# edexheim/como

Measured on AMD Instinct MI355X. Metric: GN iters/sec, 8-keyframe 640x480 photometric BA, higher is better.
Workload: dtype f64

## Files before the change

como_amd/csrc/densify.hip:

```cpp
#include "select.cuh"
#include "../../include/como_hip.h"

namespace como {

template <typename T> int select_hist(const T*, const uint8_t*, long, int, uint32_t*, int, hipStream_t);

template <typename T> struct Q4 { T x, y, z, w; };
template <typename T>
__device__ __forceinline__ Q4<T> ld4(const T* __restrict__ p) {
  Q4<T> v;
  if constexpr (sizeof(T) == 4) {
    const float4 f = *reinterpret_cast<const float4*>(p);
    v.x = f.x; v.y = f.y; v.z = f.z; v.w = f.w;
  } else {
    const double2 a = *reinterpret_cast<const double2*>(p);
    const double2 b = *reinterpret_cast<const double2*>(p + 2);
    v.x = a.x; v.y = a.y; v.z = b.x; v.w = b.y;
  }
  return v;
}

template <typename T>
__global__ __launch_bounds__(256) void dense_ref_kernel(
    const T* __restrict__ Kt, long kt_slot_stride, const int* __restrict__ pixidx, const T* __restrict__ logzm,
    const T* __restrict__ Twc, const T* __restrict__ Kmat, const T* __restrict__ dlogzm_dTwc, int n, int m, int Wimg,
    T* __restrict__ Pwn, T* __restrict__ dPwn_dTwc, T* __restrict__ uvec, T* __restrict__ zbuf, T* __restrict__ logzn_out,
    uint32_t* __restrict__ hists, const int* __restrict__ pixcoord, int compact) {
  using KeyT = typename KeyOf<T>::type;
  __shared__ uint32_t lh[SEL_BINS];
  __shared__ T coef[64][8];
  const int b = blockIdx.y;
  for (int k = threadIdx.x; k < SEL_BINS; k += 256) lh[k] = 0;
  for (int k = threadIdx.x; k < 64 * 8; k += 256) {
    const int j = k >> 3, e = k & 7;
    T v = T(0);
    if (j < m) {
      if (e == 0) v = logzm[(long)b * m + j];
      else if (e < 7) v = dlogzm_dTwc[((long)b * m + j) * 6 + (e - 1)];
    }
    coef[j][e] = v;
  }
  T Tm[12];
#pragma unroll
  for (int k = 0; k < 12; ++k) Tm[k] = Twc[16 * (long)b + k];
  const T fx = Kmat[0], fy = Kmat[4], cx = Kmat[2], cy = Kmat[5];
  __syncthreads();
  const int stride = gridDim.x * 256;
  const int iters = (n + stride - 1) / stride;
  for (int it = 0; it < iters; ++it) {
    const int i0 = it * stride + blockIdx.x * 256 + threadIdx.x;
    const bool inr = i0 < n;
    const int i = inr ? i0 : n - 1;
// ... 13 lines not shown
    const T z = exp(logz);
    const int crow = pixcoord ? pixcoord[(long)b * n + i] : row;
    T rx, ry;
    {
#pragma clang fp contract(off)
      rx = (T(crow % Wimg) - cx) / fx;
      ry = (T(crow / Wimg) - cy) / fy;
    }
    const T Xc = z * rx, Yc = z * ry, Zc = z;
    T Xw, Yw, Zw;
    rigid_apply(Tm, Xc, Yc, Zc, Xw, Yw, Zw);
    const T u0 = Tm[0] * Xc + Tm[1] * Yc + Tm[2] * Zc;
    const T u1 = Tm[4] * Xc + Tm[5] * Yc + Tm[6] * Zc;
    const T u2 = Tm[8] * Xc + Tm[9] * Yc + Tm[10] * Zc;
    if (inr && Pwn && compact) {
      const long base3 = (long)b * 3 * n + i, base6 = (long)b * 6 * n + i;
      Pwn[base3] = Xw; Pwn[base3 + n] = Yw; Pwn[base3 + 2 * (long)n] = Zw;
#pragma unroll
      for (int k = 0; k < 6; ++k) dPwn_dTwc[base6 + (long)k * n] = acc[1 + k];
    } else if (inr && Pwn) {
      const long base3 = (long)b * 3 * n + i, base18 = (long)b * 18 * n + i;
      Pwn[base3] = Xw; Pwn[base3 + n] = Yw; Pwn[base3 + 2 * (long)n] = Zw;
      uvec[base3] = u0; uvec[base3 + n] = u1; uvec[base3 + 2 * (long)n] = u2;
      const T uu[3] = {u0, u1, u2};
#pragma unroll
      for (int r = 0; r < 3; ++r) {
        const T r0 = Tm[r * 4 + 0], r1 = Tm[r * 4 + 1], r2 = Tm[r * 4 + 2];
        const T s0 = -(r1 * Zc - r2 * Yc), s1 = -(r2 * Xc - r0 * Zc), s2 = -(r0 * Yc - r1 * Xc);
        dPwn_dTwc[base18 + (long)(r * 6 + 0) * n] = s0 + uu[r] * acc[1];
        dPwn_dTwc[base18 + (long)(r * 6 + 1) * n] = s1 + uu[r] * acc[2];
        dPwn_dTwc[base18 + (long)(r * 6 + 2) * n] = s2 + uu[r] * acc[3];
        dPwn_dTwc[base18 + (long)(r * 6 + 3) * n] = r0 + uu[r] * acc[4];
        dPwn_dTwc[base18 + (long)(r * 6 + 4) * n] = r1 + uu[r] * acc[5];
        dPwn_dTwc[base18 + (long)(r * 6 + 5) * n] = r2 + uu[r] * acc[6];
      }
    }
    if (inr) {
      zbuf[(long)b * n + i] = Zc;
      if (logzn_out) logzn_out[(long)b * n + i] = logz;
    }
    sel_lds_add(lh, sel_digit<KeyT>(abs_key(Zc), 0), inr);
  }
  __syncthreads();
  if (hists) sel_flush(lh, hists + (long)b * 6 * SEL_BINS);
}

template <typename T> struct DAcc { typedef T type __attribute__((ext_vector_type(4))); };
__device__ __forceinline__ typename DAcc<float>::type d_mfma(float a, float b, typename DAcc<float>::type c) {
  return __builtin_amdgcn_mfma_f32_16x16x4f32(a, b, c, 0, 0, 0);
}
__device__ __forceinline__ typename DAcc<double>::type d_mfma(double a, double b, typename DAcc<double>::type c) {
  return __builtin_amdgcn_mfma_f64_16x16x4f64(a, b, c, 0, 0, 0);
}
template <typename T> __device__ __forceinline__ int d_mfma_row(int lane, int reg);
template <> __device__ __forceinline__ int d_mfma_row<float>(int lane, int reg) { return (lane >> 4) * 4 + reg; }
template <> __device__ __forceinline__ int d_mfma_row<double>(int lane, int reg) { return (lane >> 4) + 4 * reg; }

__device__ __forceinline__ void wave_lds_fence() {
  __builtin_amdgcn_fence(__ATOMIC_RELEASE, "workgroup");
  __builtin_amdgcn_wave_barrier();
  __builtin_amdgcn_fence(__ATOMIC_ACQUIRE, "workgroup");
}

template <typename T>
struct DRFuse {
  const int* ref_pairs;
  int np_max;
  const T* pair_T;
  const T* pair_aff;
  const T* vals;
  const T* img_base;
  const long* tgt_img;
  T* r_out;
  uint8_t* valid_out;
  uint32_t* rhists;
  int H, W, anorm_f32;
};

template <typename T, bool FUSE>
__global__ __launch_bounds__(256) void dense_ref_mfma_kernel(
    const T* __restrict__ Kt, long kt_slot_stride, const int* __restrict__ pixidx, const T* __restrict__ logzm,
    const T* __restrict__ Twc, const T* __restrict__ Kmat, const T* __restrict__ dlogzm_dTwc, int n, int m,
    int Wimg, T* __restrict__ Pwn, T* __restrict__ dPwn_dTwc, T* __restrict__ uvec, T* __restrict__ zbuf,
    T* __restrict__ logzn_out, uint32_t* __restrict__ hists, const int* __restrict__ pixcoord, int compact, DRFuse<T> fz) {
  using KeyT = typename KeyOf<T>::type;
  using acc_t = typename DAcc<T>::type;
  __shared__ uint32_t lh[SEL_BINS];
  __shared__ uint32_t lh2[FUSE ? SEL_BINS : 1];
  __shared__ T sD[4][64 * 9];
  if constexpr (FUSE) {
    for (int k = threadIdx.x; k < SEL_BINS; k += 256) lh2[k] = 0;
  }
  const int b = blockIdx.y, tid = threadIdx.x, lane = tid & 63, wv = tid >> 6, c = lane & 15, q = lane >> 4;
  for (int k = tid; k < SEL_BINS; k += 256) lh[k] = 0;
  T bop[16];
#pragma unroll
  for (int se = 0; se < 16; ++se) {
    const int k = 16 * (se >> 2) + 4 * q + (se & 3);
    T v = T(0);
    if (k < m) {
      if (c == 0) v = logzm[(long)b * m + k];
      else if (c < 7) v = dlogzm_dTwc[((long)b * m + k) * 6 + (c - 1)];
    }
    bop[se] = v;
  }
  T Tm[12];
#pragma unroll
  for (int k = 0; k < 12; ++k) Tm[k] = Twc[16 * (long)b + k];
  const T fx = Kmat[0], fy = Kmat[4], cx = Kmat[2], cy = Kmat[5];
  __syncthreads();
  T* myD = sD[wv];
  const int tiles = (n + 63) >> 6;
  Q4<T> kA[2][4], kB[2][4];
  auto load_half = [&](Q4<T> (&dst)[2][4], int tile_, int half) {
#pragma unroll
    for (int h2 = 0; h2 < 2; ++h2) {
      const int ii = min((tile_ << 6) + 16 * (2 * half + h2) + c, n - 1);
      const int rw = pixidx ? pixidx[(long)b * n + ii] : ii;
      const T* Kr = Kt + (long)b * kt_slot_stride + (long)rw * m;
#pragma unroll
      for (int s = 0; s < 4; ++s) {
        const int kk = min(16 * s + 4 * q, m - 4);
        dst[h2][s] = ld4(Kr + kk);
      }
    }
  };
  auto mma_half = [&](const Q4<T> (&src)[2][4], int half) {
#pragma unroll
    for (int h2 = 0; h2 < 2; ++h2) {
      acc_t acc = {T(0), T(0), T(0), T(0)};
#pragma unroll
      for (int s = 0; s < 4; ++s) {
        acc = d_mfma(src[h2][s].x, bop[4 * s + 0], acc);
        acc = d_mfma(src[h2][s].y, bop[4 * s + 1], acc);
        acc = d_mfma(src[h2][s].z, bop[4 * s + 2], acc);
        acc = d_mfma(src[h2][s].w, bop[4 * s + 3], acc);
      }
      if (c < 8) {
#pragma unroll
        for (int r = 0; r < 4; ++r) myD[(16 * (2 * half + h2) + d_mfma_row<T>(lane, r)) * 9 + c] = acc[r];
      }
    }
  };
  const int tstride = gridDim.x * 4;
  int tile = blockIdx.x * 4 + wv;
  if (tile < tiles) load_half(kA, tile, 0);
  for (; tile < tiles; tile += tstride) {
    const int px0 = tile << 6;
    load_half(kB, tile, 1);
    mma_half(kA, 0);
    if (tile + tstride < tiles) load_half(kA, tile + tstride, 0);
    mma_half(kB, 1);
    wave_lds_fence();
    T a7[7];
#pragma unroll
    for (int a = 0; a < 7; ++a) a7[a] = myD[lane * 9 + a];
    wave_lds_fence();
    const int i0 = px0 + lane;
    const bool inr = i0 < n;
    const int i = inr ? i0 : n - 1;
    const int row = pixidx ? pixidx[(long)b * n + i] : i;
    const T logz = a7[0];
    const T z = exp(logz);
    const int crow = pixcoord ? pixcoord[(long)b * n + i] : row;
    T rx, ry;
    {
#pragma clang fp contract(off)
      rx = (T(crow % Wimg) - cx) / fx;
      ry = (T(crow / Wimg) - cy) / fy;
    }
    const T Xc = z * rx, Yc = z * ry, Zc = z;
    T Xw, Yw, Zw;
    rigid_apply(Tm, Xc, Yc, Zc, Xw, Yw, Zw);
    const T u0 = Tm[0] * Xc + Tm[1] * Yc + Tm[2] * Zc;
    const T u1 = Tm[4] * Xc + Tm[5] * Yc + Tm[6] * Zc;
    const T u2 = Tm[8] * Xc + Tm[9] * Yc + Tm[10] * Zc;
    if (inr && Pwn && compact) {
      const long base3 = (long)b * 3 * n + i, base6 = (long)b * 6 * n + i;
      Pwn[base3] = Xw; Pwn[base3 + n] = Yw; Pwn[base3 + 2 * (long)n] = Zw;
#pragma unroll
      for (int k = 0; k < 6; ++k) dPwn_dTwc[base6 + (long)k * n] = a7[1 + k];
    } else if (inr && Pwn) {
      const long base3 = (long)b * 3 * n + i, base18 = (long)b * 18 * n + i;
      Pwn[base3] = Xw; Pwn[base3 + n] = Yw; Pwn[base3 + 2 * (long)n] = Zw;
      uvec[base3] = u0; uvec[base3 + n] = u1; uvec[base3 + 2 * (long)n] = u2;
      const T uu[3] = {u0, u1, u2};
#pragma unroll
      for (int r = 0; r < 3; ++r) {
        const T r0 = Tm[r * 4 + 0], r1 = Tm[r * 4 + 1], r2 = Tm[r * 4 + 2];
        const T s0 = -(r1 * Zc - r2 * Yc), s1 = -(r2 * Xc - r0 * Zc), s2 = -(r0 * Yc - r1 * Xc);
        dPwn_dTwc[base18 + (long)(r * 6 + 0) * n] = s0 + uu[r] * a7[1];
        dPwn_dTwc[base18 + (long)(r * 6 + 1) * n] = s1 + uu[r] * a7[2];
        dPwn_dTwc[base18 + (long)(r * 6 + 2) * n] = s2 + uu[r] * a7[3];
        dPwn_dTwc[base18 + (long)(r * 6 + 3) * n] = r0 + uu[r] * a7[4];
        dPwn_dTwc[base18 + (long)(r * 6 + 4) * n] = r1 + uu[r] * a7[5];
        dPwn_dTwc[base18 + (long)(r * 6 + 5) * n] = r2 + uu[r] * a7[6];
      }
    }
    if (inr) {
      zbuf[(long)b * n + i] = Zc;
      if (logzn_out) logzn_out[(long)b * n + i] = logz;
    }
    sel_lds_add(lh, sel_digit<KeyT>(abs_key(Zc), 0), inr);
    if constexpr (FUSE) {
      const T vr = fz.vals[(long)b * n + i];
      const T ax = fz.anorm_f32 ? (T)(1.0f / (float)fz.W) : T(1) / T(fz.W), ay = fz.anorm_f32 ? (T)(1.0f / (float)fz.H) : T(1) / T(fz.H);
      for (int q = 0; q < fz.np_max; ++q) {
        const int p = fz.ref_pairs[(long)b * fz.np_max + q];
        if (p < 0) break;
        const T* M = fz.pair_T + 12 * (long)p;
        const T scale = fz.pair_aff[2 * p], bias = fz.pair_aff[2 * p + 1];
        const T* img = fz.img_base + fz.tgt_img[p];
        T X, Y, Z;
        rigid_apply(M, Xw, Yw, Zw, X, Y, Z);
        const T pu = project1(fx, X, Z, cx);
        const T pv = project1(fy, Y, Z, cy);
        const bool ok = in_image(pu, pv, fz.H, fz.W) && (Z > T(0));
        Taps<T> t = make_taps(grid_position(pu, fz.W, ax), grid_position(pv, fz.H, ay), fz.H, fz.W);
        const T It = tap_sum(img, t);
        const T r = It - scale * vr + bias;
        if (inr) {
          const long oi = (long)p * n + i;
          fz.r_out[oi] = r;
          fz.valid_out[oi] = ok ? 1 : 0;
        }
        sel_lds_add(lh2, sel_digit<KeyT>(abs_key(r), 0), inr && ok);
      }
    }
  }
  __syncthreads();
  if (hists) sel_flush(lh, hists + (long)b * 6 * SEL_BINS);
  if constexpr (FUSE) sel_flush(lh2, fz.rhists);
}

template <typename T>
__global__ void copy_elems_kernel(const T* __restrict__ src, T* __restrict__ dst, int n) {
  const int i = blockIdx.x * blockDim.x + threadIdx.x;
  if (i < n) dst[i] = src[i];
}

template <typename T>
__global__ __launch_bounds__(256) void depth_band_kernel(
    const T* __restrict__ Kt, long kt_slot_stride, const T* __restrict__ logzm, const T* __restrict__ logzm_prev, int rows, int m,
    T* __restrict__ lref, T* __restrict__ err, T* __restrict__ l1, float* __restrict__ l1max, const T* __restrict__ med_prev3,
    T* __restrict__ zbuf, uint32_t* __restrict__ hists, unsigned* __restrict__ ncand, int init) {
  using KeyT = typename KeyOf<T>::type;
  __shared__ uint32_t lh[SEL_BINS];
  __shared__ T coef[64];
  __shared__ T sdelta, sabs;
  const int b = blockIdx.y;
  for (int k = threadIdx.x; k < SEL_BINS; k += 256) lh[k] = 0;
  if (threadIdx.x < 64) {
    const int k = threadIdx.x;
    const T cur = (k < m) ? logzm[(long)b * m + k] : T(0);
    const T prv = (k < m && !init) ? logzm_prev[(long)b * m + k] : cur;
    coef[k] = cur;
    T d = fabs(cur - prv), a = fabs(cur);
#pragma unroll
    for (int off = 32; off > 0; off >>= 1) { d = fmax(d, __shfl_xor(d, off, 64)); a = fmax(a, __shfl_xor(a, off, 64)); }
    if (k == 0) { sdelta = d; sabs = a; }
  }
  __syncthreads();
  const T eps = (sizeof(T) == 4) ? T(4e-6) : T(4e-15);
  const T delta = sdelta * (T(1) + T(64) * eps) + (sdelta > T(0) ? eps : T(0));
  const T mp = init ? T(0) : log(med_prev3[3 * b]);
  const T band = init ? T(0) : (T)l1max[b] * delta + eps * (fabs(mp) + T(1));
  const T inf = (T)__builtin_inff();
  const int stride = gridDim.x * 256;
  unsigned mycand = 0;
  float myl1max = 0.f;
  for (int i0 = blockIdx.x * 256 + threadIdx.x; i0 - (int)threadIdx.x < rows; i0 += stride) {
    const bool inr = i0 < rows;
    const int i = inr ? i0 : rows - 1;
    const long si = (long)b * rows + i;
    bool cand = init != 0;
    T e = T(0), lr = T(0), rl1 = T(0);
    if (!init) {
      rl1 = l1[si];
      lr = lref[si];
      e = err[si] + rl1 * delta;
      cand = !((lr + e < mp - band) || (lr - e > mp + band));
    }
    T z;
    if (cand) {
      const T* Kr = Kt + (long)b * kt_slot_stride + (long)i * m;
      T acc = T(0), s1 = T(0);
// ... 185 lines not shown
  using acc_t = typename KAcc<T>::type;
  __shared__ T sK[64 * 65];
  __shared__ T sx[64 * 2];
  __shared__ T sE[64 * 4];
  const int b = blockIdx.y;
  for (int k = threadIdx.x; k < 64 * 64; k += 256) {
    const int r = k >> 6, c = k & 63;
    sK[r * 65 + c] = (r < m && c < m) ? Kinv[(long)b * m * m + (long)r * m + c] : T(0);
  }
  for (int k = threadIdx.x; k < 64 * 2; k += 256) sx[k] = (k < m * 2) ? xm[(long)b * m * 2 + k] : T(0);
  for (int k = threadIdx.x; k < 64 * 4; k += 256) sE[k] = (k < m * 4) ? Em[(long)b * m * 4 + k] : ((k & 3) == 0 || (k & 3) == 3 ? T(1) : T(0));
  __syncthreads();
  const long np = (long)Hp * Wp;
  const T ar = T(1) / T(Hc), ac = T(1) / T(Wc);
  const int lane = threadIdx.x & 63, wv = threadIdx.x >> 6, px = lane & 15, kq = lane >> 4;
  const long groups = (np + 15) / 16;
  for (long grp = (long)blockIdx.x * 4 + wv; grp < groups; grp += (long)gridDim.x * 4) {
    const long p = min(grp * 16 + px, np - 1);
    const int row = (int)(p / Wp), col = (int)(p % Wp);
    T rn, cn;
    {
#pragma clang fp contract(off)
      rn = (T(2) * ar) * T(row) + ar - T(1);
      cn = (T(2) * ac) * T(col) + ac - T(1);
    }
    T En[4];
    cov_lookup(cov + (long)b * 4 * Hc * Wc, Hc, Wc, rn, cn, En);
    T a[16];
#pragma unroll
    for (int s2 = 0; s2 < 16; ++s2) {
      const int k = 4 * s2 + kq;
      const T v = kernel_py(rn, cn, En, sx[2 * k], sx[2 * k + 1], sE + 4 * k) * scale;
      a[s2] = (k < m) ? v : T(0);
    }
#pragma unroll
    for (int t = 0; t < 4; ++t) {
      if (16 * t >= m) break;
      acc_t acc = {T(0), T(0), T(0), T(0)};
#pragma unroll
      for (int s2 = 0; s2 < 16; ++s2) acc = k_mfma(a[s2], sK[(4 * s2 + kq) * 65 + 16 * t + px], acc);
      const int j = 16 * t + px;
#pragma unroll
      for (int r = 0; r < 4; ++r) {
        const long pr = grp * 16 + k_mfma_row<T>(lane, r);
        if (pr < np && j < m) {
          out[((long)b * np + pr) * m + j] = acc[r];
          if (out32) out32[((long)b * np + pr) * m + j] = (float)acc[r];
        }
      }
    }
  }
}

template <typename T>
int dense_ref(const T* Kt, long kt_slot_stride, const int* pixidx, const T* logzm, const T* Twc, const T* Kmat,
              const T* dlogzm_dTwc, int B, int n, int m, int Wimg, T* Pwn, T* dPwn_dTwc, T* uvec, T* zbuf, T* logzn_out,
              void* hists_v, T* med_out3, const int* pixcoord, int flags, hipStream_t s, const DRFuse<T>* fuse = nullptr) {
  using KeyT = typename KeyOf<T>::type;
  const int compact = (flags & 16) ? 1 : 0;
  const bool depth_only = (flags & 8) != 0;
  if (!Kt || !logzm || !Twc || !Kmat || !dlogzm_dTwc || !zbuf || !hists_v || !med_out3 ||
      B <= 0 || n <= 0 || m <= 0 || m > 64 || (m & 3) || Wimg <= 0)
    return COMO_ERR_ARG;
  if (depth_only) { Pwn = nullptr; dPwn_dTwc = nullptr; uvec = nullptr; }
  else if (!Pwn || !dPwn_dTwc || (!uvec && !compact)) return COMO_ERR_ARG;
  uint32_t* hists = (uint32_t*)hists_v;
  if (!(flags & 4)) {
  if ((flags & 64) && (flags & 2)) hists = nullptr;
  if (hists && !(flags & 1) && !zero_words(hists, (size_t)B * 6 * SEL_BINS, s))
    return COMO_ERR_LAUNCH;
  int gx = (n + 255) / 256;
  if (gx > 512) gx = 512;
  if (sizeof(T) == 4 || (!depth_only && !(flags & 32))) {
    int gm = ((n + 63) / 64 + 3) / 4;
    if (gm > 256) gm = 256;
    if (fuse && !depth_only)
      hipLaunchKernelGGL((dense_ref_mfma_kernel<T, true>), dim3(gm, B), dim3(256), 0, s, Kt, kt_slot_stride, pixidx, logzm, Twc, Kmat,
                         dlogzm_dTwc, n, m, Wimg, Pwn, dPwn_dTwc, uvec, zbuf, logzn_out, hists, pixcoord, compact, *fuse);
    else
      hipLaunchKernelGGL((dense_ref_mfma_kernel<T, false>), dim3(gm, B), dim3(256), 0, s, Kt, kt_slot_stride, pixidx, logzm, Twc, Kmat,
                         dlogzm_dTwc, n, m, Wimg, Pwn, dPwn_dTwc, uvec, zbuf, logzn_out, hists, pixcoord, compact, DRFuse<T>{});
  } else {
    if (fuse) return COMO_ERR_ARG;
    hipLaunchKernelGGL(dense_ref_kernel<T>, dim3(gx, B), dim3(256), 0, s, Kt, kt_slot_stride, pixidx, logzm, Twc, Kmat,
                       dlogzm_dTwc, n, m, Wimg, Pwn, dPwn_dTwc, uvec, zbuf, logzn_out, hists, pixcoord, compact);
  }
  COMO_CHECK_LAUNCH();
  }
  if (flags & 2) return COMO_OK;
  for (int p = 1; p < SelCfg<KeyT>::NPASS; ++p) {
    int rc = select_hist<T>(zbuf, nullptr, n, B, hists, p | 0x100, s);
    if (rc) return rc;
  }
  return COMO_OK;
}

}

extern "C" {

int como_select_finish_f32(const void*, int, float*, como_stream_t);
int como_select_finish_f64(const void*, int, double*, como_stream_t);

int como_dense_ref_f32(const float* Kt, long kt_slot_stride, const int* pixidx, const float* logzm, const float* Twc,
                       const float* K, const float* dlogzm_dTwc, int B, int n, int m, int Wimg, float* Pwn,
                       float* dPwn_dTwc, float* uvec, float* zbuf, float* logzn_out, void* hists, float* med_out3,
                       const int* pixcoord, int flags, como_stream_t stream) {
  int rc = como::dense_ref<float>(Kt, kt_slot_stride, pixidx, logzm, Twc, K, dlogzm_dTwc, B, n, m, Wimg, Pwn, dPwn_dTwc, uvec,
                                  zbuf, logzn_out, hists, med_out3, pixcoord, flags, (hipStream_t)stream);
  if (rc || (flags & 2)) return rc;
  return como_select_finish_f32(hists, B, med_out3, stream);
}
int como_dense_ref_f64(const double* Kt, long kt_slot_stride, const int* pixidx, const double* logzm, const double* Twc,
                       const double* K, const double* dlogzm_dTwc, int B, int n, int m, int Wimg, double* Pwn,
                       double* dPwn_dTwc, double* uvec, double* zbuf, double* logzn_out, void* hists, double* med_out3,
                       const int* pixcoord, int flags, como_stream_t stream) {
  int rc = como::dense_ref<double>(Kt, kt_slot_stride, pixidx, logzm, Twc, K, dlogzm_dTwc, B, n, m, Wimg, Pwn, dPwn_dTwc, uvec,
                                   zbuf, logzn_out, hists, med_out3, pixcoord, flags, (hipStream_t)stream);
  if (rc || (flags & 2)) return rc;
  return como_select_finish_f64(hists, B, med_out3, stream);
}

#define COMO_DEF_DR_FUSED(SFX, T)                                                                                               \
  int como_dense_ref_fused_##SFX(const T* Kt, long kt_slot_stride, const int* pixidx, const T* logzm, const T* Twc, const T* K,   \
                                 const T* dlogzm_dTwc, int B, int n, int m, int Wimg, T* Pwn, T* dPwn_dTwc, T* uvec, T* zbuf,     \
                                 T* logzn_out, void* hists, T* med_out3, const int* pixcoord, int flags, const como_dr_fuse* f,   \
                                 como_stream_t stream) {                                                                        \
    if (!f || !f->ref_pairs || f->np_max <= 0 || !f->pair_T || !f->pair_aff || !f->vals || !f->img_base || !f->tgt_img ||        \
        !f->r_out || !f->valid_out || !f->rhists || f->H < 3 || f->W < 3 || (flags & (4 | 8)))                                  \
      return COMO_ERR_ARG;                                                                                                      \
    como::DRFuse<T> fz{f->ref_pairs, f->np_max, (const T*)f->pair_T, (const T*)f->pair_aff, (const T*)f->vals,                   \
                       (const T*)f->img_base, f->tgt_img, (T*)f->r_out, (uint8_t*)f->valid_out, (uint32_t*)f->rhists, f->H, f->W,  \
                       f->anorm_f32};                                                                                           \
    int rc = como::dense_ref<T>(Kt, kt_slot_stride, pixidx, logzm, Twc, K, dlogzm_dTwc, B, n, m, Wimg, Pwn, dPwn_dTwc, uvec, zbuf, \
// ... 135 lines not shown
```

como_amd/odom/backend/dense_ref.py:

```python
import torch

from como_amd import _lib

_ws = {}


def dense_reference_planes(Kt, n, compact, ws=None):
    dt, dev = Kt.dtype, Kt.device
    B = Kt.shape[0]
    key = (str(dev), dt, B, n) if not compact else (str(dev), dt, B, n, "compact")
    own = ws
    w = own.get(key) if own is not None else _ws.get(key)
    if w is None:
        w = {"Pwn": torch.empty((B, 3, n), device=dev, dtype=dt),
             "dT": torch.empty((B, 6 if compact else 18, n), device=dev, dtype=dt),
             "uvec": None if compact else torch.empty((B, 3, n), device=dev, dtype=dt),
             "z": torch.empty((B, n), device=dev, dtype=dt),
             "logz": torch.empty((B, n), device=dev, dtype=dt), "med": torch.empty((B, 3), device=dev, dtype=dt),
             "hists": torch.empty((B * _lib.lib().como_select_workspace_bytes() // 4,), device=dev, dtype=torch.int32)}
        if own is not None:
            own[key] = w
        else:
            _ws.clear()
            _ws[key] = w
    return w


def dense_reference_factored(logzm, Twc, Kt, pixidx, K, dlogzm_dTwc, Wimg, want_logz=True, med_out=None, pixcoord=None,
                             hists=None, ws=None, part="all", compact=False, fuse=None, call_cache=None, stream=None):
    if call_cache is not None:
        ent = call_cache.get(("dr", part))
        if ent is not None:
            fn, args, fz, out = ent
            st = stream if stream is not None else _lib.stream_ptr(Kt.device)
            rc = fn(*args, fz, st) if fz is not None else fn(*args, st)
            _lib.check(rc, "como_dense_ref")
            return out
    _lib.require_cuda(logzm, Twc, Kt, K, dlogzm_dTwc)
    dt, dev = Kt.dtype, Kt.device
    B, rows, m = Kt.shape
    n = pixidx.shape[1] if pixidx is not None else rows
    L = _lib.lib()
    ws = dense_reference_planes(Kt, n, compact, ws)
    med = med_out if med_out is not None else ws["med"]
    lz = logzm.reshape(B, m).to(dt).contiguous()
    dl = dlogzm_dTwc.reshape(B, m, 6).to(dt).contiguous()
    Tw = Twc.to(dt).contiguous()
    Kc = K.to(dt).contiguous()
    flags = (1 if hists is not None else 0) | {"all": 0, "points": 2, "median": 4}[part] | (16 if compact else 0)
    args = (Kt.data_ptr(), Kt.stride(0), _lib.ptr(pixidx), lz.data_ptr(), Tw.data_ptr(), Kc.data_ptr(), dl.data_ptr(), B, n, m,
            int(Wimg), ws["Pwn"].data_ptr(), ws["dT"].data_ptr(), _lib.ptr(ws["uvec"]), ws["z"].data_ptr(),
            ws["logz"].data_ptr() if want_logz else None, (hists if hists is not None else ws["hists"]).data_ptr(), med.data_ptr(),
            _lib.ptr(pixcoord), flags)
    st = stream if stream is not None else _lib.stream_ptr(dev)
    out = (ws["Pwn"], ws["dT"], ws["uvec"], med[:, 0], ws["logz"])
    if fuse is not None and part != "median":
        import ctypes
        fn, fz = getattr(L, "como_dense_ref_fused_" + _lib.suffix(dt)), ctypes.byref(fuse)
        rc = fn(*args, fz, st)
    else:
        fn, fz = getattr(L, "como_dense_ref_" + _lib.suffix(dt)), None
        rc = fn(*args, st)
    _lib.check(rc, "como_dense_ref")
    if call_cache is not None:
        call_cache[("dr", part)] = (fn, args, fz, out)
        call_cache[("dr_keep", part)] = (lz, dl, Tw, Kc, ws, med, fuse, hists, pixidx, pixcoord, Kt)
    return out


_di_ws = {}


def depth_image(Kt, logzm, out=None, logz_out=None):
    _lib.require_cuda(Kt, logzm)
    dt, dev = Kt.dtype, Kt.device
    B, rows, m = Kt.shape
    if Kt.stride(2) != 1 or Kt.stride(1) != m:
        Kt = Kt.contiguous()
    L = _lib.lib()
    key = (str(dev), torch.cuda.current_stream(dev).cuda_stream, dt, B, m)
    w = _di_ws.get(key)
    if w is None:
        w = _di_ws[key] = {"hists": torch.zeros((B * L.como_select_workspace_bytes() // 4,), device=dev, dtype=torch.int32),
                           "eye": torch.eye(4, device=dev, dtype=dt).repeat(B, 1, 1).contiguous(),
                           "K": torch.eye(3, device=dev, dtype=dt), "dl": torch.zeros((B, m, 6), device=dev, dtype=dt),
                           "med": torch.zeros((B, 3), device=dev, dtype=dt)}
    z = out if out is not None else torch.empty((B, rows), device=dev, dtype=dt)
    lz = logzm.reshape(B, m)
    if lz.dtype != dt or not lz.is_contiguous():
        lz = lz.to(dt).contiguous()
    rc = getattr(L, "como_dense_ref_" + _lib.suffix(dt))(
        Kt.data_ptr(), Kt.stride(0), None, lz.data_ptr(), w["eye"].data_ptr(), w["K"].data_ptr(), w["dl"].data_ptr(), B, rows, m, 1,
        None, None, None, z.data_ptr(), _lib.ptr(logz_out), w["hists"].data_ptr(), w["med"].data_ptr(), None, 8 | 2 | 64, _lib.stream_ptr(dev))
    _lib.check(rc, "como_dense_ref (depth image)")
    return z


BAND_MEDIAN = __import__("os").environ.get("COMO_BAND_MEDIAN", "1") != "0"


def full_image_median(logzm, Kt, med_out, ws, hists=None, part="all", reduce=None, band=None, reduce_max=None, call_cache=None,
                      stream=None):
# ... 98 lines not shown
```

Measured before the change: 816.3.

## Cache per-pair constants in LDS and size dense_ref grid to resident occupancy

Up to eight per-pair transform, affine and image-offset constants are staged into shared memory once per block, so the fused residual loop no longer reloads them from global memory for every pixel. Pairs beyond the cap fall back to global loads. The grid size of the MFMA dense_ref kernel is now derived from queried occupancy (resident blocks per CU times CU count, split across keyframes) when there are enough tiles, instead of a fixed cap of 256. This trades some launch-shape heuristics and a cached one-time occupancy query for fewer redundant loads and less grid tail or oversubscription.

```diff
diff --git a/como_amd/csrc/densify.hip b/como_amd/csrc/densify.hip
--- a/como_amd/csrc/densify.hip
+++ b/como_amd/csrc/densify.hip
@@ -142,6 +142,15 @@
   int H, W, anorm_f32;
 };
 
+constexpr int DR_PAIR_CAP = 8;
+template <typename T>
+struct DRPairConst {
+  T M[12];
+  T scale, bias;
+  long img;
+  int p;
+};
+
 template <typename T, bool FUSE>
 __global__ __launch_bounds__(256) void dense_ref_mfma_kernel(
     const T* __restrict__ Kt, long kt_slot_stride, const int* __restrict__ pixidx, const T* __restrict__ logzm,
@@ -153,10 +162,21 @@
   __shared__ uint32_t lh[SEL_BINS];
   __shared__ uint32_t lh2[FUSE ? SEL_BINS : 1];
   __shared__ T sD[4][64 * 9];
+  __shared__ DRPairConst<T> spc[FUSE ? DR_PAIR_CAP : 1];
+  const int b = blockIdx.y, tid = threadIdx.x, lane = tid & 63, wv = tid >> 6, c = lane & 15, q = lane >> 4;
   if constexpr (FUSE) {
     for (int k = threadIdx.x; k < SEL_BINS; k += 256) lh2[k] = 0;
-  }
-  const int b = blockIdx.y, tid = threadIdx.x, lane = tid & 63, wv = tid >> 6, c = lane & 15, q = lane >> 4;
+    if (tid < 16 * DR_PAIR_CAP) {
+      const int slot = tid >> 4, e = tid & 15;
+      const int p = (slot < fz.np_max) ? fz.ref_pairs[(long)b * fz.np_max + slot] : -1;
+      DRPairConst<T>& pc = spc[slot];
+      if (e < 12) pc.M[e] = (p >= 0) ? fz.pair_T[12 * (long)p + e] : T(0);
+      else if (e == 12) pc.scale = (p >= 0) ? fz.pair_aff[2 * p] : T(0);
+      else if (e == 13) pc.bias = (p >= 0) ? fz.pair_aff[2 * p + 1] : T(0);
+      else if (e == 14) pc.img = (p >= 0) ? fz.tgt_img[p] : 0L;
+      else pc.p = p;
+    }
+  }
   for (int k = tid; k < SEL_BINS; k += 256) lh[k] = 0;
   T bop[16];
 #pragma unroll
@@ -270,12 +290,7 @@
     if constexpr (FUSE) {
       const T vr = fz.vals[(long)b * n + i];
       const T ax = fz.anorm_f32 ? (T)(1.0f / (float)fz.W) : T(1) / T(fz.W), ay = fz.anorm_f32 ? (T)(1.0f / (float)fz.H) : T(1) / T(fz.H);
-      for (int q = 0; q < fz.np_max; ++q) {
-        const int p = fz.ref_pairs[(long)b * fz.np_max + q];
-        if (p < 0) break;
-        const T* M = fz.pair_T + 12 * (long)p;
-        const T scale = fz.pair_aff[2 * p], bias = fz.pair_aff[2 * p + 1];
-        const T* img = fz.img_base + fz.tgt_img[p];
+      auto pair_pass = [&](int p, const T* M, const T& scale, const T& bias, const T* img) {
         T X, Y, Z;
         rigid_apply(M, Xw, Yw, Zw, X, Y, Z);
         const T pu = project1(fx, X, Z, cx);
@@ -290,6 +305,20 @@
           fz.valid_out[oi] = ok ? 1 : 0;
         }
         sel_lds_add(lh2, sel_digit<KeyT>(abs_key(r), 0), inr && ok);
+      };
+      const int nlds = min(fz.np_max, DR_PAIR_CAP);
+      int q = 0;
+      for (; q < nlds; ++q) {
+        const DRPairConst<T>& pc = spc[q];
+        if (pc.p < 0) break;
+        pair_pass(pc.p, pc.M, pc.scale, pc.bias, fz.img_base + pc.img);
+      }
+      if (q == DR_PAIR_CAP) {
+        for (; q < fz.np_max; ++q) {
+          const int p = fz.ref_pairs[(long)b * fz.np_max + q];
+          if (p < 0) break;
+          pair_pass(p, fz.pair_T + 12 * (long)p, fz.pair_aff[2 * p], fz.pair_aff[2 * p + 1], fz.img_base + fz.tgt_img[p]);
+        }
       }
     }
   }
@@ -588,6 +617,20 @@
   }
 }
 
+struct DRResident { int blocks, cus; };
+template <typename T, bool FUSE>
+const DRResident& dense_ref_resident() {
+  static const DRResident r = [] {
+    int dev = 0, cus = 0, per_cu = 0;
+    if (hipGetDevice(&dev) != hipSuccess ||
+        hipDeviceGetAttribute(&cus, hipDeviceAttributeMultiprocessorCount, dev) != hipSuccess ||
+        hipOccupancyMaxActiveBlocksPerMultiprocessor(&per_cu, dense_ref_mfma_kernel<T, FUSE>, 256, 0) != hipSuccess)
+      return DRResident{0, 0};
+    return DRResident{per_cu * cus, cus};
+  }();
+  return r;
+}
+
 template <typename T>
 int dense_ref(const T* Kt, long kt_slot_stride, const int* pixidx, const T* logzm, const T* Twc, const T* Kmat,
               const T* dlogzm_dTwc, int B, int n, int m, int Wimg, T* Pwn, T* dPwn_dTwc, T* uvec, T* zbuf, T* logzn_out,
@@ -608,9 +651,16 @@
   int gx = (n + 255) / 256;
   if (gx > 512) gx = 512;
   if (sizeof(T) == 4 || (!depth_only && !(flags & 32))) {
-    int gm = ((n + 63) / 64 + 3) / 4;
-    if (gm > 256) gm = 256;
-    if (fuse && !depth_only)
+    const bool fused = fuse && !depth_only;
+    const DRResident res = fused ? dense_ref_resident<T, true>() : dense_ref_resident<T, false>();
+    if (res.blocks <= 0) return COMO_ERR_LAUNCH;
+    const int tiles = (n + 63) / 64;
+    int gm = (tiles + 3) / 4;
+    const int per_kf = res.blocks / B, one_per_cu = (res.cus + B - 1) / B;
+    const int want = per_kf > one_per_cu ? per_kf : one_per_cu;
+    if (tiles >= 16 * want) gm = want;
+    else if (gm > 256) gm = 256;
+    if (fused)
       hipLaunchKernelGGL((dense_ref_mfma_kernel<T, true>), dim3(gm, B), dim3(256), 0, s, Kt, kt_slot_stride, pixidx, logzm, Twc, Kmat,
                          dlogzm_dTwc, n, m, Wimg, Pwn, dPwn_dTwc, uvec, zbuf, logzn_out, hists, pixcoord, compact, *fuse);
     else
```

New measurement: 820.8 (median of 4 runs). About the same (+0.5%).

## Prefetch pixel row indices, cache pair poses in LDS, add occupancy hint

Applied to the files above, without the earlier changes.

The dense reference MFMA kernel now loads pixel row indices once per tile, one per lane, and shuffles them across the wave instead of reloading them per 16-lane group. The next tile's indices are prefetched two iterations ahead, and the fused residual values are loaded earlier to overlap with the MFMA work. In the fused path, the first few pair poses, affine terms and image offsets are staged in shared memory so they are not re-read from global memory for every pixel. The kernel also gains a launch-bounds occupancy hint and an optional 4x4x4 f64 MFMA variant that is compiled only under a build flag; the hint may raise register pressure.

```diff
diff --git a/como_amd/csrc/densify.hip b/como_amd/csrc/densify.hip
--- a/como_amd/csrc/densify.hip
+++ b/como_amd/csrc/densify.hip
@@ -117,6 +117,7 @@
 __device__ __forceinline__ typename DAcc<double>::type d_mfma(double a, double b, typename DAcc<double>::type c) {
   return __builtin_amdgcn_mfma_f64_16x16x4f64(a, b, c, 0, 0, 0);
 }
+__device__ __forceinline__ double d_mfma4(double a, double b, double c) { return __builtin_amdgcn_mfma_f64_4x4x4f64(a, b, c, 0, 0, 0); }
 template <typename T> __device__ __forceinline__ int d_mfma_row(int lane, int reg);
 template <> __device__ __forceinline__ int d_mfma_row<float>(int lane, int reg) { return (lane >> 4) * 4 + reg; }
 template <> __device__ __forceinline__ int d_mfma_row<double>(int lane, int reg) { return (lane >> 4) + 4 * reg; }
@@ -142,32 +143,54 @@
   int H, W, anorm_f32;
 };
 
-template <typename T, bool FUSE>
-__global__ __launch_bounds__(256) void dense_ref_mfma_kernel(
+constexpr int DR_PAIRS_LDS = 8;
+template <typename T, bool FUSE, bool M4>
+__device__ __forceinline__ void dense_ref_mfma_body(
     const T* __restrict__ Kt, long kt_slot_stride, const int* __restrict__ pixidx, const T* __restrict__ logzm,
     const T* __restrict__ Twc, const T* __restrict__ Kmat, const T* __restrict__ dlogzm_dTwc, int n, int m,
     int Wimg, T* __restrict__ Pwn, T* __restrict__ dPwn_dTwc, T* __restrict__ uvec, T* __restrict__ zbuf,
-    T* __restrict__ logzn_out, uint32_t* __restrict__ hists, const int* __restrict__ pixcoord, int compact, DRFuse<T> fz) {
+    T* __restrict__ logzn_out, uint32_t* __restrict__ hists, const int* __restrict__ pixcoord, int compact, const DRFuse<T>& fz) {
+  static_assert(!M4 || sizeof(T) == 8, "the 4x4x4 shape is the float64 form");
   using KeyT = typename KeyOf<T>::type;
   using acc_t = typename DAcc<T>::type;
+  constexpr int NPC = DR_PAIRS_LDS;
   __shared__ uint32_t lh[SEL_BINS];
   __shared__ uint32_t lh2[FUSE ? SEL_BINS : 1];
   __shared__ T sD[4][64 * 9];
+  __shared__ T sPair[FUSE ? NPC : 1][16];
+  __shared__ long sImg[FUSE ? NPC : 1];
+  __shared__ int sPid[FUSE ? NPC : 1];
+  const int b = blockIdx.y, tid = threadIdx.x, lane = tid & 63, wv = tid >> 6, c = lane & 15, q = lane >> 4;
   if constexpr (FUSE) {
-    for (int k = threadIdx.x; k < SEL_BINS; k += 256) lh2[k] = 0;
-  }
-  const int b = blockIdx.y, tid = threadIdx.x, lane = tid & 63, wv = tid >> 6, c = lane & 15, q = lane >> 4;
+    for (int k = tid; k < SEL_BINS; k += 256) lh2[k] = 0;
+    for (int k = tid; k < NPC * 16; k += 256) {
+      const int pq = k >> 4, e = k & 15;
+      const int p = pq < fz.np_max ? fz.ref_pairs[(long)b * fz.np_max + pq] : -1;
+      T v = T(0);
+      if (p >= 0 && e < 12) v = fz.pair_T[12 * (long)p + e];
+      else if (p >= 0 && e < 14) v = fz.pair_aff[2 * p + (e - 12)];
+      sPair[pq][e] = v;
+      if (e == 0) {
+        sPid[pq] = p;
+        sImg[pq] = p >= 0 ? fz.tgt_img[p] : 0;
+      }
+    }
+  }
   for (int k = tid; k < SEL_BINS; k += 256) lh[k] = 0;
-  T bop[16];
+  T bop[M4 ? 32 : 16];
 #pragma unroll
   for (int se = 0; se < 16; ++se) {
     const int k = 16 * (se >> 2) + 4 * q + (se & 3);
-    T v = T(0);
-    if (k < m) {
-      if (c == 0) v = logzm[(long)b * m + k];
-      else if (c < 7) v = dlogzm_dTwc[((long)b * m + k) * 6 + (c - 1)];
-    }
-    bop[se] = v;
+#pragma unroll
+    for (int g = 0; g < (M4 ? 2 : 1); ++g) {
+      const int col = M4 ? 4 * g + (c & 3) : c;
+      T v = T(0);
+      if (k < m) {
+        if (col == 0) v = logzm[(long)b * m + k];
+        else if (col < 7) v = dlogzm_dTwc[((long)b * m + k) * 6 + (col - 1)];
+      }
+      bop[16 * g + se] = v;
+    }
   }
   T Tm[12];
 #pragma unroll
@@ -177,11 +200,14 @@
   T* myD = sD[wv];
   const int tiles = (n + 63) >> 6;
   Q4<T> kA[2][4], kB[2][4];
-  auto load_half = [&](Q4<T> (&dst)[2][4], int tile_, int half) {
+  auto tile_rows = [&](int tile_) -> int {
+    const int ii = min((tile_ << 6) + lane, n - 1);
+    return pixidx ? pixidx[(long)b * n + ii] : ii;
+  };
+  auto load_half = [&](Q4<T> (&dst)[2][4], int rows, int half) {
 #pragma unroll
     for (int h2 = 0; h2 < 2; ++h2) {
-      const int ii = min((tile_ << 6) + 16 * (2 * half + h2) + c, n - 1);
-      const int rw = pixidx ? pixidx[(long)b * n + ii] : ii;
+      const int rw = __shfl(rows, 16 * (2 * half + h2) + c, 64);
       const T* Kr = Kt + (long)b * kt_slot_stride + (long)rw * m;
 #pragma unroll
       for (int s = 0; s < 4; ++s) {
@@ -191,43 +217,73 @@
     }
   };
   auto mma_half = [&](const Q4<T> (&src)[2][4], int half) {
-#pragma unroll
-    for (int h2 = 0; h2 < 2; ++h2) {
-      acc_t acc = {T(0), T(0), T(0), T(0)};
+    if constexpr (M4) {
+      T lo[2] = {T(0), T(0)}, hi[2] = {T(0), T(0)};
 #pragma unroll
       for (int s = 0; s < 4; ++s) {
-        acc = d_mfma(src[h2][s].x, bop[4 * s + 0], acc);
-        acc = d_mfma(src[h2][s].y, bop[4 * s + 1], acc);
-        acc = d_mfma(src[h2][s].z, bop[4 * s + 2], acc);
-        acc = d_mfma(src[h2][s].w, bop[4 * s + 3], acc);
-      }
-      if (c < 8) {
-#pragma unroll
-        for (int r = 0; r < 4; ++r) myD[(16 * (2 * half + h2) + d_mfma_row<T>(lane, r)) * 9 + c] = acc[r];
+#pragma unroll
+        for (int e = 0; e < 4; ++e) {
+#pragma unroll
+          for (int h2 = 0; h2 < 2; ++h2) {
+            const T a = e == 0 ? src[h2][s].x : e == 1 ? src[h2][s].y : e == 2 ? src[h2][s].z : src[h2][s].w;
+            lo[h2] = d_mfma4(a, bop[4 * s + e], lo[h2]);
+            hi[h2] = d_mfma4(a, bop[16 + 4 * s + e], hi[h2]);
+          }
+        }
+      }
+#pragma unroll
+      for (int h2 = 0; h2 < 2; ++h2) {
+        T* d = myD + (16 * (2 * half + h2) + 4 * (c >> 2) + q) * 9 + (c & 3);
+        d[0] = lo[h2];
+        d[4] = hi[h2];
+      }
+    } else {
+#pragma unroll
+      for (int h2 = 0; h2 < 2; ++h2) {
+        acc_t acc = {T(0), T(0), T(0), T(0)};
+#pragma unroll
+        for (int s = 0; s < 4; ++s) {
+          acc = d_mfma(src[h2][s].x, bop[4 * s + 0], acc);
+          acc = d_mfma(src[h2][s].y, bop[4 * s + 1], acc);
+          acc = d_mfma(src[h2][s].z, bop[4 * s + 2], acc);
+          acc = d_mfma(src[h2][s].w, bop[4 * s + 3], acc);
+        }
+        if (c < 8) {
+#pragma unroll
+          for (int r = 0; r < 4; ++r) myD[(16 * (2 * half + h2) + d_mfma_row<T>(lane, r)) * 9 + c] = acc[r];
+        }
       }
     }
   };
   const int tstride = gridDim.x * 4;
   int tile = blockIdx.x * 4 + wv;
-  if (tile < tiles) load_half(kA, tile, 0);
+  int rows0 = 0, rows1 = 0;
+  if (tile < tiles) rows0 = tile_rows(tile);
+  if (tile + tstride < tiles) rows1 = tile_rows(tile + tstride);
+  if (tile < tiles) load_half(kA, rows0, 0);
   for (; tile < tiles; tile += tstride) {
     const int px0 = tile << 6;
-    load_half(kB, tile, 1);
-    mma_half(kA, 0);
-    if (tile + tstride < tiles) load_half(kA, tile + tstride, 0);
-    mma_half(kB, 1);
-    wave_lds_fence();
-    T a7[7];
-#pragma unroll
-    for (int a = 0; a < 7; ++a) a7[a] = myD[lane * 9 + a];
-    wave_lds_fence();
     const int i0 = px0 + lane;
     const bool inr = i0 < n;
     const int i = inr ? i0 : n - 1;
-    const int row = pixidx ? pixidx[(long)b * n + i] : i;
+    const int crow = pixcoord ? pixcoord[(long)b * n + i] : rows0;
+    T vr = T(0);
+    if constexpr (FUSE) vr = fz.vals[(long)b * n + i];
+    load_half(kB, rows0, 1);
+    mma_half(kA, 0);
+    int rows2 = 0;
+    if (tile + tstride < tiles) load_half(kA, rows1, 0);
+    if (tile + 2 * tstride < tiles) rows2 = tile_rows(tile + 2 * tstride);
+    mma_half(kB, 1);
+    rows0 = rows1;
+    rows1 = rows2;
+    wave_lds_fence();
+    T a7[7];
+#pragma unroll
+    for (int a = 0; a < 7; ++a) a7[a] = myD[lane * 9 + a];
+    wave_lds_fence();
     const T logz = a7[0];
     const T z = exp(logz);
-    const int crow = pixcoord ? pixcoord[(long)b * n + i] : row;
     T rx, ry;
     {
 #pragma clang fp contract(off)
@@ -268,14 +324,28 @@
     }
     sel_lds_add(lh, sel_digit<KeyT>(abs_key(Zc), 0), inr);
     if constexpr (FUSE) {
-      const T vr = fz.vals[(long)b * n + i];
       const T ax = fz.anorm_f32 ? (T)(1.0f / (float)fz.W) : T(1) / T(fz.W), ay = fz.anorm_f32 ? (T)(1.0f / (float)fz.H) : T(1) / T(fz.H);
-      for (int q = 0; q < fz.np_max; ++q) {
-        const int p = fz.ref_pairs[(long)b * fz.np_max + q];
-        if (p < 0) break;
-        const T* M = fz.pair_T + 12 * (long)p;
-        const T scale = fz.pair_aff[2 * p], bias = fz.pair_aff[2 * p + 1];
-        const T* img = fz.img_base + fz.tgt_img[p];
+      for (int pq = 0; pq < fz.np_max; ++pq) {
+        int p;
+        T M[12], scale, bias;
+        const T* img;
+        if (pq < NPC) {
+          p = __builtin_amdgcn_readfirstlane(sPid[pq]);
+          if (p < 0) break;
+#pragma unroll
+          for (int k = 0; k < 12; ++k) M[k] = sPair[pq][k];
+          scale = sPair[pq][12];
+          bias = sPair[pq][13];
+          img = fz.img_base + sImg[pq];
+        } else {
+          p = fz.ref_pairs[(long)b * fz.np_max + pq];
+          if (p < 0) break;
+#pragma unroll
+          for (int k = 0; k < 12; ++k) M[k] = fz.pair_T[12 * (long)p + k];
+          scale = fz.pair_aff[2 * p];
+          bias = fz.pair_aff[2 * p + 1];
+          img = fz.img_base + fz.tgt_img[p];
+        }
         T X, Y, Z;
         rigid_apply(M, Xw, Yw, Zw, X, Y, Z);
         const T pu = project1(fx, X, Z, cx);
@@ -297,6 +367,25 @@
   if (hists) sel_flush(lh, hists + (long)b * 6 * SEL_BINS);
   if constexpr (FUSE) sel_flush(lh2, fz.rhists);
 }
+
+#define DR_MFMA_PARAMS                                                                                                         \
+  const T *__restrict__ Kt, long kt_slot_stride, const int *__restrict__ pixidx, const T *__restrict__ logzm,                  \
+      const T *__restrict__ Twc, const T *__restrict__ Kmat, const T *__restrict__ dlogzm_dTwc, int n, int m, int Wimg,        \
+      T *__restrict__ Pwn, T *__restrict__ dPwn_dTwc, T *__restrict__ uvec, T *__restrict__ zbuf, T *__restrict__ logzn_out,   \
+      uint32_t *__restrict__ hists, const int *__restrict__ pixcoord, int compact, DRFuse<T> fz
+#define DR_MFMA_ARGS \
+  Kt, kt_slot_stride, pixidx, logzm, Twc, Kmat, dlogzm_dTwc, n, m, Wimg, Pwn, dPwn_dTwc, uvec, zbuf, logzn_out, hists, pixcoord, compact, fz
+
+template <typename T, bool FUSE>
+__global__ __launch_bounds__(256, sizeof(T) == 4 ? 4 : 2) void dense_ref_mfma_kernel(DR_MFMA_PARAMS) {
+  dense_ref_mfma_body<T, FUSE, false>(DR_MFMA_ARGS);
+}
+#ifdef COMO_AB_VARIANTS
+template <typename T, bool FUSE>
+__global__ __launch_bounds__(256, 2) void dense_ref_mfma4_kernel(DR_MFMA_PARAMS) {
+  dense_ref_mfma_body<T, FUSE, sizeof(T) == 8>(DR_MFMA_ARGS);
+}
+#endif
 
 template <typename T>
 __global__ void copy_elems_kernel(const T* __restrict__ src, T* __restrict__ dst, int n) {
@@ -610,12 +699,17 @@
   if (sizeof(T) == 4 || (!depth_only && !(flags & 32))) {
     int gm = ((n + 63) / 64 + 3) / 4;
     if (gm > 256) gm = 256;
-    if (fuse && !depth_only)
-      hipLaunchKernelGGL((dense_ref_mfma_kernel<T, true>), dim3(gm, B), dim3(256), 0, s, Kt, kt_slot_stride, pixidx, logzm, Twc, Kmat,
-                         dlogzm_dTwc, n, m, Wimg, Pwn, dPwn_dTwc, uvec, zbuf, logzn_out, hists, pixcoord, compact, *fuse);
-    else
-      hipLaunchKernelGGL((dense_ref_mfma_kernel<T, false>), dim3(gm, B), dim3(256), 0, s, Kt, kt_slot_stride, pixidx, logzm, Twc, Kmat,
-                         dlogzm_dTwc, n, m, Wimg, Pwn, dPwn_dTwc, uvec, zbuf, logzn_out, hists, pixcoord, compact, DRFuse<T>{});
+    const bool fused = fuse && !depth_only;
+    const DRFuse<T> fz = fused ? *fuse : DRFuse<T>{};
+    auto kern = fused ? dense_ref_mfma_kernel<T, true> : dense_ref_mfma_kernel<T, false>;
+#ifdef COMO_AB_VARIANTS
+    if constexpr (sizeof(T) == 8) {
+      static const bool m4 = [] { const char* e = getenv("COMO_DR_MFMA4"); return e && e[0] == '1'; }();
+      if (m4) kern = fused ? dense_ref_mfma4_kernel<T, true> : dense_ref_mfma4_kernel<T, false>;
+    }
+#endif
+    hipLaunchKernelGGL(kern, dim3(gm, B), dim3(256), 0, s, Kt, kt_slot_stride, pixidx, logzm, Twc, Kmat, dlogzm_dTwc, n, m, Wimg,
+                       Pwn, dPwn_dTwc, uvec, zbuf, logzn_out, hists, pixcoord, compact, fz);
   } else {
     if (fuse) return COMO_ERR_ARG;
     hipLaunchKernelGGL(dense_ref_kernel<T>, dim3(gx, B), dim3(256), 0, s, Kt, kt_slot_stride, pixidx, logzm, Twc, Kmat,
```

Measured after the change: 828.1 before, 835.4 after (median of 6 runs). No clear change (+0.9%).

## Prefetch pixel indices, stage pair params in LDS, size grid by occupancy

Applied to the files above, without the earlier changes.

Reworks the fused dense-reference MFMA kernel. Each pair's transform, affine and image offset are staged once in shared memory and broadcast wave-uniformly. Pixel-index rows are prefetched two tiles ahead and distributed with shuffles instead of per-lane reloads, and for f64 two pairs' bilinear taps are issued together to overlap gathers. The tile loop is specialized by compile-time tags, and the grid is sized from the occupancy API (resident blocks / B) with an optional cap from Python. This adds code complexity, extra register pressure from the prefetch, and an occupancy query on first launch.

```diff
diff --git a/como_amd/csrc/densify.hip b/como_amd/csrc/densify.hip
--- a/como_amd/csrc/densify.hip
+++ b/como_amd/csrc/densify.hip
@@ -1,3 +1,6 @@
+#include <map>
+#include <mutex>
+#include <type_traits>
 #include "select.cuh"
 #include "../../include/como_hip.h"
 
@@ -127,6 +130,13 @@
   __builtin_amdgcn_fence(__ATOMIC_ACQUIRE, "workgroup");
 }
 
+__device__ __forceinline__ float wave_uniform(float v) {
+  return __int_as_float(__builtin_amdgcn_readfirstlane(__float_as_int(v)));
+}
+__device__ __forceinline__ double wave_uniform(double v) {
+  return __hiloint2double(__builtin_amdgcn_readfirstlane(__double2hiint(v)), __builtin_amdgcn_readfirstlane(__double2loint(v)));
+}
+
 template <typename T>
 struct DRFuse {
   const int* ref_pairs;
@@ -142,6 +152,8 @@
   int H, W, anorm_f32;
 };
 
+constexpr int DR_NPQ = 4;
+
 template <typename T, bool FUSE>
 __global__ __launch_bounds__(256) void dense_ref_mfma_kernel(
     const T* __restrict__ Kt, long kt_slot_stride, const int* __restrict__ pixidx, const T* __restrict__ logzm,
@@ -153,10 +165,25 @@
   __shared__ uint32_t lh[SEL_BINS];
   __shared__ uint32_t lh2[FUSE ? SEL_BINS : 1];
   __shared__ T sD[4][64 * 9];
+  __shared__ T sPC[FUSE ? DR_NPQ : 1][16];
+  __shared__ long sImg[FUSE ? DR_NPQ : 1];
+  __shared__ int sPid[FUSE ? DR_NPQ : 1];
+  const int b = blockIdx.y, tid = threadIdx.x, lane = tid & 63, wv = tid >> 6, c = lane & 15, q = lane >> 4;
   if constexpr (FUSE) {
     for (int k = threadIdx.x; k < SEL_BINS; k += 256) lh2[k] = 0;
-  }
-  const int b = blockIdx.y, tid = threadIdx.x, lane = tid & 63, wv = tid >> 6, c = lane & 15, q = lane >> 4;
+    if (tid < DR_NPQ * 16) {
+      const int pq = tid >> 4, e = tid & 15;
+      const int p = pq < fz.np_max ? fz.ref_pairs[(long)b * fz.np_max + pq] : -1;
+      T v = T(0);
+      if (p >= 0) {
+        if (e < 12) v = fz.pair_T[12 * (long)p + e];
+        else if (e < 14) v = fz.pair_aff[2 * p + (e - 12)];
+        else if (e == 14) sImg[pq] = fz.tgt_img[p];
+      }
+      sPC[pq][e] = v;
+      if (e == 15) sPid[pq] = p;
+    }
+  }
   for (int k = tid; k < SEL_BINS; k += 256) lh[k] = 0;
   T bop[16];
 #pragma unroll
@@ -177,12 +204,24 @@
   T* myD = sD[wv];
   const int tiles = (n + 63) >> 6;
   Q4<T> kA[2][4], kB[2][4];
-  auto load_half = [&](Q4<T> (&dst)[2][4], int tile_, int half) {
+  const int* __restrict__ pidx = pixidx ? pixidx : pixcoord;
+  const int* __restrict__ pcrd = pixcoord ? pixcoord : pixidx;
+  auto tile_rows = [&](int tile_) { return pidx[(long)b * n + min((tile_ << 6) + lane, n - 1)]; };
+  auto load_half = [&](Q4<T> (&dst)[2][4], int tile_, int half, int rows_reg, auto pix_tag) {
+    constexpr bool PIX = decltype(pix_tag)::value;
+    int rw[2];
 #pragma unroll
     for (int h2 = 0; h2 < 2; ++h2) {
-      const int ii = min((tile_ << 6) + 16 * (2 * half + h2) + c, n - 1);
-      const int rw = pixidx ? pixidx[(long)b * n + ii] : ii;
-      const T* Kr = Kt + (long)b * kt_slot_stride + (long)rw * m;
+      const int pl = 16 * (2 * half + h2) + c;
+      rw[h2] = min((tile_ << 6) + pl, n - 1);
+      if constexpr (PIX) {
+        const int v = __shfl(rows_reg, pl, 64);
+        rw[h2] = pixidx ? v : rw[h2];
+      }
+    }
+#pragma unroll
+    for (int h2 = 0; h2 < 2; ++h2) {
+      const T* Kr = Kt + (long)b * kt_slot_stride + (long)rw[h2] * m;
 #pragma unroll
       for (int s = 0; s < 4; ++s) {
         const int kk = min(16 * s + 4 * q, m - 4);
@@ -207,27 +246,45 @@
       }
     }
   };
-  const int tstride = gridDim.x * 4;
-  int tile = blockIdx.x * 4 + wv;
-  if (tile < tiles) load_half(kA, tile, 0);
-  for (; tile < tiles; tile += tstride) {
+  int np = 0;
+  if constexpr (FUSE) {
+    while (np < fz.np_max && (np < DR_NPQ ? sPid[np] : fz.ref_pairs[(long)b * fz.np_max + np]) >= 0) ++np;
+    np = __builtin_amdgcn_readfirstlane(np);
+  }
+  T ax = T(0), ay = T(0);
+  if constexpr (FUSE) {
+    ax = fz.anorm_f32 ? (T)(1.0f / (float)fz.W) : T(1) / T(fz.W);
+    ay = fz.anorm_f32 ? (T)(1.0f / (float)fz.H) : T(1) / T(fz.H);
+  }
+  const int tend = tiles, tstep = gridDim.x * 4, tfirst = blockIdx.x * 4 + wv;
+  int rows_cur = 0, rows_next = 0;
+  auto tile_body = [&](const int tile, auto pix_tag, auto more_tag) {
+    constexpr bool PIX = decltype(pix_tag)::value, MORE = decltype(more_tag)::value;
     const int px0 = tile << 6;
-    load_half(kB, tile, 1);
+    const int i0 = px0 + lane;
+    const bool inr = i0 < n;
+    const int i = inr ? i0 : n - 1;
+    int row = i, crow = i, rows_after = 0;
+    if constexpr (PIX) {
+      rows_after = tile_rows(tile + 2 * tstep);
+      const int cv = pcrd[(long)b * n + i];
+      row = pixidx ? rows_cur : i;
+      crow = pixcoord ? cv : row;
+    }
+    T vr = T(0);
+    if constexpr (FUSE) vr = fz.vals[(long)b * n + i];
+    load_half(kB, tile, 1, rows_cur, pix_tag);
     mma_half(kA, 0);
-    if (tile + tstride < tiles) load_half(kA, tile + tstride, 0);
+    if constexpr (MORE) load_half(kA, tile + tstep, 0, rows_next, pix_tag);
+    if constexpr (PIX) { rows_cur = rows_next; rows_next = rows_after; }
     mma_half(kB, 1);
     wave_lds_fence();
     T a7[7];
 #pragma unroll
     for (int a = 0; a < 7; ++a) a7[a] = myD[lane * 9 + a];
     wave_lds_fence();
-    const int i0 = px0 + lane;
-    const bool inr = i0 < n;
-    const int i = inr ? i0 : n - 1;
-    const int row = pixidx ? pixidx[(long)b * n + i] : i;
     const T logz = a7[0];
     const T z = exp(logz);
-    const int crow = pixcoord ? pixcoord[(long)b * n + i] : row;
     T rx, ry;
     {
 #pragma clang fp contract(off)
@@ -268,31 +325,63 @@
     }
     sel_lds_add(lh, sel_digit<KeyT>(abs_key(Zc), 0), inr);
     if constexpr (FUSE) {
-      const T vr = fz.vals[(long)b * n + i];
-      const T ax = fz.anorm_f32 ? (T)(1.0f / (float)fz.W) : T(1) / T(fz.W), ay = fz.anorm_f32 ? (T)(1.0f / (float)fz.H) : T(1) / T(fz.H);
-      for (int q = 0; q < fz.np_max; ++q) {
-        const int p = fz.ref_pairs[(long)b * fz.np_max + q];
-        if (p < 0) break;
-        const T* M = fz.pair_T + 12 * (long)p;
-        const T scale = fz.pair_aff[2 * p], bias = fz.pair_aff[2 * p + 1];
-        const T* img = fz.img_base + fz.tgt_img[p];
+      struct PairTaps { Taps<T> t; const T* img; T scale, bias; int p; bool ok; };
+      auto pair_taps = [&](int pq) {
+        PairTaps o;
+        T M[12];
+        if (pq < DR_NPQ) {
+#pragma unroll
+          for (int e = 0; e < 12; ++e) M[e] = wave_uniform(sPC[pq][e]);
+          o.scale = wave_uniform(sPC[pq][12]); o.bias = wave_uniform(sPC[pq][13]);
+          o.img = fz.img_base + sImg[pq];
+          o.p = sPid[pq];
+        } else {
+          o.p = fz.ref_pairs[(long)b * fz.np_max + pq];
+#pragma unroll
+          for (int e = 0; e < 12; ++e) M[e] = fz.pair_T[12 * (long)o.p + e];
+          o.scale = fz.pair_aff[2 * o.p]; o.bias = fz.pair_aff[2 * o.p + 1];
+          o.img = fz.img_base + fz.tgt_img[o.p];
+        }
         T X, Y, Z;
         rigid_apply(M, Xw, Yw, Zw, X, Y, Z);
         const T pu = project1(fx, X, Z, cx);
         const T pv = project1(fy, Y, Z, cy);
-        const bool ok = in_image(pu, pv, fz.H, fz.W) && (Z > T(0));
-        Taps<T> t = make_taps(grid_position(pu, fz.W, ax), grid_position(pv, fz.H, ay), fz.H, fz.W);
-        const T It = tap_sum(img, t);
-        const T r = It - scale * vr + bias;
+        o.ok = in_image(pu, pv, fz.H, fz.W) && (Z > T(0));
+        o.t = make_taps(grid_position(pu, fz.W, ax), grid_position(pv, fz.H, ay), fz.H, fz.W);
+        return o;
+      };
+      auto pair_out = [&](const PairTaps& o, T It) {
+        const T r = It - o.scale * vr + o.bias;
         if (inr) {
-          const long oi = (long)p * n + i;
+          const long oi = (long)o.p * n + i;
           fz.r_out[oi] = r;
-          fz.valid_out[oi] = ok ? 1 : 0;
+          fz.valid_out[oi] = o.ok ? 1 : 0;
         }
-        sel_lds_add(lh2, sel_digit<KeyT>(abs_key(r), 0), inr && ok);
-      }
-    }
-  }
+        sel_lds_add(lh2, sel_digit<KeyT>(abs_key(r), 0), inr && o.ok);
+      };
+      constexpr int PSTEP = sizeof(T) == 8 ? 2 : 1;
+      for (int pq = 0; pq < np; pq += PSTEP) {
+        if (PSTEP == 2 && pq + 1 < np) {
+          const PairTaps o0 = pair_taps(pq), o1 = pair_taps(pq + 1);
+          const T It0 = tap_sum(o0.img, o0.t), It1 = tap_sum(o1.img, o1.t);
+          pair_out(o0, It0);
+          pair_out(o1, It1);
+        } else {
+          const PairTaps o0 = pair_taps(pq);
+          pair_out(o0, tap_sum(o0.img, o0.t));
+        }
+      }
+    }
+  };
+  auto run = [&](auto pix_tag) {
+    int tile = tfirst;
+    if constexpr (decltype(pix_tag)::value) { rows_cur = tile_rows(tile); rows_next = tile_rows(tile + tstep); }
+    if (tile < tend) load_half(kA, tile, 0, rows_cur, pix_tag);
+    for (; tile + tstep < tend; tile += tstep) tile_body(tile, pix_tag, std::true_type{});
+    if (tile < tend) tile_body(tile, pix_tag, std::false_type{});
+  };
+  if (pixidx || pixcoord) run(std::true_type{});
+  else run(std::false_type{});
   __syncthreads();
   if (hists) sel_flush(lh, hists + (long)b * 6 * SEL_BINS);
   if constexpr (FUSE) sel_flush(lh2, fz.rhists);
@@ -588,6 +677,22 @@
   }
 }
 
+static int dr_resident(const void* kernel) {
+  static std::mutex mu;
+  static std::map<const void*, int> known;
+  std::lock_guard<std::mutex> lock(mu);
+  auto it = known.find(kernel);
+  if (it != known.end()) return it->second;
+  int dev = 0, ncu = 0, occ = 0, res = 0;
+  if (hipGetDevice(&dev) == hipSuccess && hipDeviceGetAttribute(&ncu, hipDeviceAttributeMultiprocessorCount, dev) == hipSuccess &&
+      hipOccupancyMaxActiveBlocksPerMultiprocessor(&occ, kernel, 256, 0) == hipSuccess && ncu > 0 && occ > 0)
+    res = ncu * occ;
+  else
+    (void)hipGetLastError();
+  if (res > 0) known[kernel] = res;
+  return res;
+}
+
 template <typename T>
 int dense_ref(const T* Kt, long kt_slot_stride, const int* pixidx, const T* logzm, const T* Twc, const T* Kmat,
               const T* dlogzm_dTwc, int B, int n, int m, int Wimg, T* Pwn, T* dPwn_dTwc, T* uvec, T* zbuf, T* logzn_out,
@@ -608,9 +713,16 @@
   int gx = (n + 255) / 256;
   if (gx > 512) gx = 512;
   if (sizeof(T) == 4 || (!depth_only && !(flags & 32))) {
-    int gm = ((n + 63) / 64 + 3) / 4;
-    if (gm > 256) gm = 256;
-    if (fuse && !depth_only)
+    const bool fused = fuse && !depth_only;
+    const int resident = fused ? dr_resident((const void*)dense_ref_mfma_kernel<T, true>)
+                               : dr_resident((const void*)dense_ref_mfma_kernel<T, false>);
+    if (resident < 1) return COMO_ERR_LAUNCH;
+    int gm = resident / B;
+    const int gcap = (flags >> 16) & 0x7fff;
+    if (gm > ((n + 63) / 64 + 3) / 4) gm = ((n + 63) / 64 + 3) / 4;
+    if (gcap && gm > gcap) gm = gcap;
+    if (gm < 1) gm = 1;
+    if (fused)
       hipLaunchKernelGGL((dense_ref_mfma_kernel<T, true>), dim3(gm, B), dim3(256), 0, s, Kt, kt_slot_stride, pixidx, logzm, Twc, Kmat,
                          dlogzm_dTwc, n, m, Wimg, Pwn, dPwn_dTwc, uvec, zbuf, logzn_out, hists, pixcoord, compact, *fuse);
     else
diff --git a/como_amd/odom/backend/dense_ref.py b/como_amd/odom/backend/dense_ref.py
--- a/como_amd/odom/backend/dense_ref.py
+++ b/como_amd/odom/backend/dense_ref.py
@@ -3,6 +3,7 @@
 from como_amd import _lib
 
 _ws = {}
+_MAX_WORKGROUPS = 0
 
 
 def dense_reference_planes(Kt, n, compact, ws=None):
@@ -47,7 +48,8 @@
     dl = dlogzm_dTwc.reshape(B, m, 6).to(dt).contiguous()
     Tw = Twc.to(dt).contiguous()
     Kc = K.to(dt).contiguous()
-    flags = (1 if hists is not None else 0) | {"all": 0, "points": 2, "median": 4}[part] | (16 if compact else 0)
+    flags = ((1 if hists is not None else 0) | {"all": 0, "points": 2, "median": 4}[part] | (16 if compact else 0) |
+             (min(max(int(_MAX_WORKGROUPS), 0), 0x7fff) << 16))
     args = (Kt.data_ptr(), Kt.stride(0), _lib.ptr(pixidx), lz.data_ptr(), Tw.data_ptr(), Kc.data_ptr(), dl.data_ptr(), B, n, m,
             int(Wimg), ws["Pwn"].data_ptr(), ws["dT"].data_ptr(), _lib.ptr(ws["uvec"]), ws["z"].data_ptr(),
             ws["logz"].data_ptr() if want_logz else None, (hists if hists is not None else ws["hists"]).data_ptr(), med.data_ptr(),
```

Result: no change. 813.1 before, 816.5 after, median of 6 (+0.4%).
